# elisabeth96/nerf-rs

Hardware: AMD Instinct MI355X
Metric: rays/sec, lego 800x800 (64 coarse + 128 fine samples per ray) (higher is better)
Workload: dtype f32

## Files before the change

### bindings/rust/nerf-mi355x-sys/src/lib.rs

```rust
#![allow(non_camel_case_types)]
use std::os::raw::{c_char, c_int, c_void};

#[repr(C)]
pub struct nerf_ctx {
    _private: [u8; 0],
}

#[repr(C)]
#[derive(Clone, Copy, Debug, Default)]
pub struct nerf_camera {
    pub nx: i32,
    pub ny: i32,
    pub alpha_width: f32,
    pub alpha_height: f32,
    pub pos: [f32; 3],
    pub dir: [f32; 3],
    pub up: [f32; 3],
    pub near: f32,
    pub far: f32,
}

pub const NERF_MLP_F32: i32 = 0;
pub const NERF_MLP_BF16: i32 = 1;
pub const NERF_MLP_BF16X3: i32 = 2;
// ... 102 lines not shown
    pub fn nerf_pack_network_dir(dir: *const c_char, blob_path: *const c_char) -> c_int;
    pub fn nerf_load_network_blob(ctx: *mut nerf_ctx, which: c_int, blob_path: *const c_char) -> c_int;
    pub fn nerf_debug_pack_network_dir(dir: *const c_char, wstream: *mut f32, wstream_cap: usize, small: *mut f32,
                                       small_cap: usize, wstream_len: *mut usize, small_len: *mut usize) -> c_int;
    pub fn nerf_debug_fold_network_dir(dir: *const c_char, wstream: *mut f32, wstream_cap: usize, small: *mut f32,
                                       small_cap: usize, wstream_len: *mut usize, small_len: *mut usize) -> c_int;
    pub fn nerf_debug_network_stream_dir(dir: *const c_char, kind: c_int, out: *mut u16, cap: usize, n: *mut usize, available: *mut c_int) -> c_int;
    pub fn nerf_debug_zero_skip_network_dir(dir: *const c_char, eligible: *mut c_int) -> c_int;
    pub fn nerf_debug_split_bf16x3(values: *const f32, n: usize, parts: *mut u16) -> c_int;
    pub fn nerf_debug_split_f16x2(values: *const f32, n: usize, parts: *mut u16) -> c_int;
    pub fn nerf_debug_certify_policy(margin: f32, audited: u64, violations: u64, headroom: f32, max_error: f32, new_margin: *mut f32) -> c_int;
    pub fn nerf_debug_ray_grouping(n_rays: c_int, samples_per_ray: c_int, enabled: c_int, first_slot_of_wave_tile: *mut i32) -> c_int;
    pub fn nerf_debug_wave_tiling(rows: c_int, rays_per_row: c_int, samples_per_ray: c_int, full: c_int, ray_grouping: c_int, wave_tiling: c_int,
                                  slot: *mut i32) -> c_int;
    pub fn nerf_debug_tile_rotation(n_tiles: c_int, n_workgroups: c_int, rotation: c_int, workgroup_of_tile: *mut i32, round_of_tile: *mut i32) -> c_int;
    pub fn nerf_debug_shader_clock_mhz(ctx: *mut nerf_ctx, mhz: *mut f64) -> c_int;
    pub fn nerf_debug_workgroup_clocks(ctx: *mut nerf_ctx, out: *mut u64, n_workgroups: usize) -> c_int;
    pub fn nerf_forward_batch(ctx: *mut nerf_ctx, which: c_int, pts_soa: *const f32, dirs_aos: *const f32, n: usize,
                              rgb_aos: *mut f32, sigma: *mut f32) -> c_int;
    pub fn nerf_forward_batch_ex(ctx: *mut nerf_ctx, which: c_int, mlp_dtype: c_int, pts_soa: *const f32, dirs_aos: *const f32,
                                 n: usize, rgb_aos: *mut f32, sigma: *mut f32) -> c_int;
    pub fn nerf_forward_batch_device(ctx: *mut nerf_ctx, which: c_int, d_pts_soa: *const f32, d_dirs_aos: *const f32,
                                     n: usize, d_rgb_aos: *mut f32, d_sigma: *mut f32, stream: *mut c_void) -> c_int;
    pub fn nerf_density_batch(ctx: *mut nerf_ctx, which: c_int, pts_soa: *const f32, n: usize, sigma: *mut f32) -> c_int;
    pub fn nerf_density_batch_device(ctx: *mut nerf_ctx, which: c_int, d_pts_soa: *const f32, n: usize, d_sigma: *mut f32,
                                     stream: *mut c_void) -> c_int;
    pub fn nerf_density_grid(ctx: *mut nerf_ctx, which: c_int, lo: *const f32, step: *const f32, dims: *const i32, sigma_out: *mut f32,
                             threshold: f32, occ_bits: *mut u32, n_occupied: *mut u64, bounds: *mut i32) -> c_int;
    pub fn nerf_density_grid_device(ctx: *mut nerf_ctx, which: c_int, lo: *const f32, step: *const f32, dims: *const i32,
                                    d_sigma_out: *mut f32, threshold: f32, d_occ_bits: *mut u32, n_occupied: *mut u64, bounds: *mut i32,
// ... 176 lines not shown
```

### include/nerf_mi355x.h

```cpp
#ifndef NERF_MI355X_H
#define NERF_MI355X_H

#include <stddef.h>
#include <stdint.h>

#ifdef __cplusplus
extern "C" {
#endif

typedef struct nerf_ctx nerf_ctx;

typedef enum {
    NERF_OK = 0,
    NERF_ERR_INVALID = -1,
    NERF_ERR_IO = -2,
    NERF_ERR_MISSING = -3,
    NERF_ERR_SHAPE = -4,
    NERF_ERR_HIP = -5,
    NERF_ERR_STATE = -6,
    NERF_ERR_PARSE = -7
} nerf_status;

enum { NERF_NET_COARSE = 0, NERF_NET_FINE = 1 };
enum { NERF_MLP_F32 = 0, NERF_MLP_BF16 = 1, NERF_MLP_BF16X3 = 2, NERF_MLP_F16X2 = 3 };
// ... 58 lines not shown
int nerf_check_network_dir(const char *dir);
int nerf_check_network_blob(const char *blob_path);
int nerf_debug_pack_network_dir(const char *dir, float *wstream, size_t wstream_cap, float *small, size_t small_cap,
                                size_t *wstream_len, size_t *small_len);
int nerf_debug_fold_network_dir(const char *dir, float *wstream, size_t wstream_cap, float *small, size_t small_cap,
                                size_t *wstream_len, size_t *small_len);
enum { NERF_STREAM_BF16V2 = 0, NERF_STREAM_F16V2 = 1, NERF_STREAM_BF16X3 = 2, NERF_STREAM_F16X2 = 3 };
int nerf_debug_network_stream_dir(const char *dir, int kind, uint16_t *out, size_t cap, size_t *n, int *available);
int nerf_debug_zero_skip_network_dir(const char *dir, int *eligible);
int nerf_debug_split_bf16x3(const float *values, size_t n, uint16_t *parts );
int nerf_debug_certify_policy(float margin, uint64_t audited, uint64_t violations, float headroom, float max_error, float *new_margin);
int nerf_debug_split_f16x2(const float *values, size_t n, uint16_t *parts );
int nerf_debug_ray_grouping(int n_rays, int samples_per_ray, int enabled, int32_t *first_slot_of_wave_tile);
int nerf_debug_wave_tiling(int rows, int rays_per_row, int samples_per_ray, int full, int ray_grouping, int wave_tiling, int32_t *slot);
int nerf_debug_tile_rotation(int n_tiles, int n_workgroups, int rotation, int32_t *workgroup_of_tile, int32_t *round_of_tile);

int nerf_forward_batch(nerf_ctx *ctx, int which, const float *pts_soa , const float *dirs_aos ,
                       size_t n, float *rgb_aos , float *sigma );
int nerf_forward_batch_ex(nerf_ctx *ctx, int which, int mlp_dtype, const float *pts_soa, const float *dirs_aos, size_t n,
                          float *rgb_aos, float *sigma);
int nerf_forward_batch_device(nerf_ctx *ctx, int which, const float *d_pts_soa, const float *d_dirs_aos, size_t n,
                              float *d_rgb_aos, float *d_sigma, void *stream);

int nerf_density_batch(nerf_ctx *ctx, int which, const float *pts_soa , size_t n, float *sigma );
int nerf_density_batch_device(nerf_ctx *ctx, int which, const float *d_pts_soa, size_t n, float *d_sigma, void *stream);
int nerf_density_grid(nerf_ctx *ctx, int which, const float lo[3], const float step[3], const int32_t dims[3], float *sigma_out,
                      float threshold, uint32_t *occ_bits, uint64_t *n_occupied, int32_t bounds[6]);
int nerf_density_grid_device(nerf_ctx *ctx, int which, const float lo[3], const float step[3], const int32_t dims[3],
                             float *d_sigma_out, float threshold, uint32_t *d_occ_bits, uint64_t *n_occupied, int32_t bounds[6],
                             void *stream);
// ... 192 lines not shown
```

### nerf-rs_amd/_lib.py

```python
import ctypes as C
import os
import subprocess

_HERE = os.path.dirname(os.path.abspath(__file__))
_LIB = None

f32p = C.POINTER(C.c_float)
u8p = C.POINTER(C.c_uint8)
u32p = C.POINTER(C.c_uint32)
i32p = C.POINTER(C.c_int32)


class NerfError(RuntimeError):

    def __init__(self, code, msg):
        super().__init__(f"[{code}] {msg}")
        self.code = code
        self.msg = msg


class CCamera(C.Structure):
    _fields_ = [("nx", C.c_int32), ("ny", C.c_int32), ("alpha_width", C.c_float), ("alpha_height", C.c_float),
                ("pos", C.c_float * 3), ("dir", C.c_float * 3), ("up", C.c_float * 3),
                ("near", C.c_float), ("far", C.c_float)]
# ... 42 lines not shown
                                        C.POINTER(CCamera)]),
    "nerf_check_network_dir": (C.c_int, [C.c_char_p]),
    "nerf_check_network_blob": (C.c_int, [C.c_char_p]),
    "nerf_debug_pack_network_dir": (C.c_int, [C.c_char_p, f32p, C.c_size_t, f32p, C.c_size_t, C.POINTER(C.c_size_t),
                                              C.POINTER(C.c_size_t)]),
    "nerf_debug_fold_network_dir": (C.c_int, [C.c_char_p, f32p, C.c_size_t, f32p, C.c_size_t, C.POINTER(C.c_size_t),
                                              C.POINTER(C.c_size_t)]),
    "nerf_debug_network_stream_dir": (C.c_int, [C.c_char_p, C.c_int, C.POINTER(C.c_uint16), C.c_size_t, C.POINTER(C.c_size_t),
                                                C.POINTER(C.c_int)]),
    "nerf_debug_zero_skip_network_dir": (C.c_int, [C.c_char_p, C.POINTER(C.c_int)]),
    "nerf_debug_split_bf16x3": (C.c_int, [f32p, C.c_size_t, C.POINTER(C.c_uint16)]),
    "nerf_debug_split_f16x2": (C.c_int, [f32p, C.c_size_t, C.POINTER(C.c_uint16)]),
    "nerf_debug_certify_policy": (C.c_int, [C.c_float, C.c_uint64, C.c_uint64, C.c_float, C.c_float, f32p]),
    "nerf_debug_ray_grouping": (C.c_int, [C.c_int, C.c_int, C.c_int, C.POINTER(C.c_int32)]),
    "nerf_debug_tile_rotation": (C.c_int, [C.c_int, C.c_int, C.c_int, C.POINTER(C.c_int32), C.POINTER(C.c_int32)]),
    "nerf_debug_wave_tiling": (C.c_int, [C.c_int, C.c_int, C.c_int, C.c_int, C.c_int, C.c_int, C.POINTER(C.c_int32)]),
    "nerf_forward_batch": (C.c_int, [C.c_void_p, C.c_int, f32p, f32p, C.c_size_t, f32p, f32p]),
    "nerf_forward_batch_ex": (C.c_int, [C.c_void_p, C.c_int, C.c_int, f32p, f32p, C.c_size_t, f32p, f32p]),
    "nerf_forward_batch_device": (C.c_int, [C.c_void_p, C.c_int, C.c_void_p, C.c_void_p, C.c_size_t, C.c_void_p,
                                            C.c_void_p, C.c_void_p]),
    "nerf_density_batch": (C.c_int, [C.c_void_p, C.c_int, f32p, C.c_size_t, f32p]),
    "nerf_density_batch_device": (C.c_int, [C.c_void_p, C.c_int, C.c_void_p, C.c_size_t, C.c_void_p, C.c_void_p]),
    "nerf_density_grid": (C.c_int, [C.c_void_p, C.c_int, f32p, f32p, i32p, f32p, C.c_float, u32p, C.POINTER(C.c_uint64), i32p]),
    "nerf_density_grid_device": (C.c_int, [C.c_void_p, C.c_int, f32p, f32p, i32p, C.c_void_p, C.c_float, C.c_void_p,
                                           C.POINTER(C.c_uint64), i32p, C.c_void_p]),
    "nerf_isosurface_grid": (C.c_int, [C.c_void_p, f32p, f32p, f32p, i32p, C.c_float, f32p, f32p, C.c_size_t, u32p, C.c_size_t,
                                       C.POINTER(C.c_uint64), C.POINTER(C.c_uint64)]),
    "nerf_extract_mesh": (C.c_int, [C.c_void_p, C.c_int, f32p, f32p, i32p, C.c_float, f32p, f32p, f32p, C.c_size_t, u32p, C.c_size_t,
                                    C.POINTER(C.c_uint64), C.POINTER(C.c_uint64)]),
    "nerf_extract_mesh_device": (C.c_int, [C.c_void_p, C.c_int, f32p, f32p, i32p, C.c_float, C.c_void_p, C.c_void_p, C.c_void_p, C.c_size_t,
# ... 130 lines not shown
```

### nerf-rs_amd/csrc/mlp_kernel.h

```cpp
#pragma once
#include <hip/hip_runtime.h>

#include "mlp_layout.h"

enum { MLP_MODE_POINTS = 0, MLP_MODE_RAYS = 1, MLP_MODE_LIST = 2, MLP_MODE_GRID = 3 };

struct MlpArgs {
    const float *wstream;
    const float *small_params;
    int n_points;
    int mode;
    const float *pts_soa;
    const float *dirs_aos;
    const float *ray_dirs;
    const float *t;
    int samples_per_ray;
    float origin[3];
    float *sigma_out;
    float *rgb_out;
    int skip_empty;
    unsigned long long *skip_counter;
    unsigned long long *clock_out;
    unsigned int *nonfinite;
    int raw_pre;
// ... 4 lines not shown
    int grid_n[3];
    float occ_threshold;
    unsigned int *occ_bits;
    int zero_skip;
    unsigned long long *zskip_stats;
    int ray_grouping;
    int wave_tiling;
    int rays_per_row;
    nerfmlp::RayLaunchMap ray_map;
    const float *ray_origins;
    int depth_order;
    const unsigned int *order_table;
    int order_tiles, order_points;
    int tile_rotation;
    int empty_vote;
};

inline nerfmlp::DepthOrder nerf_mlp_depth_order(const MlpArgs &a, bool full) {
    return nerfmlp::depth_order_of(a.n_points, a.samples_per_ray, a.rays_per_row, full,
                                   a.mode == MLP_MODE_RAYS && a.depth_order != 0 && a.wave_tiling != 0 && a.skip_empty == 0);
}

hipError_t nerf_mlp_init();
hipError_t nerf_mlp_launch(const MlpArgs &a, bool full, int n_blocks, hipStream_t stream);
hipError_t nerf_zskip_clear(unsigned long long *stats, hipStream_t stream);
hipError_t nerf_zskip_print(const char *what, unsigned long long *stats, hipStream_t stream);
hipError_t nerf_mlp_bf16v2_init();
hipError_t nerf_mlp_bf16v2_launch(const MlpArgs &a, bool full, int n_blocks, hipStream_t stream);
hipError_t nerf_prefilter_f16v2_init();
hipError_t nerf_mlp_f16v2_launch(const MlpArgs &a, int n_blocks, hipStream_t stream);
struct SeqArgs;
// ... 57 lines not shown
```

### nerf-rs_amd/csrc/mlp_kernel.hip

```cpp
#include <hip/hip_runtime.h>
#include <stdint.h>
#include <stdio.h>

#include "mlp_f32_core.hip.h"
#include "mlp_kernel.h"

using namespace nerfmlp;
using namespace mlpdev;

using namespace mlpf32;

template <bool FULL, int MODE>
__global__ __launch_bounds__(256, 1) void nerf_mlp_kernel(const MlpArgs A) {
    extern __shared__ __attribute__((aligned(16))) char smem[];
    const LDS_AS char *lds = (const LDS_AS char *)smem;
    const LDS_AS float *small = (const LDS_AS float *)(lds + kRingSlots * kChunkBytes);

    const int tid = threadIdx.x;
    const int lane = tid & 63;
    const int wave = __builtin_amdgcn_readfirstlane(tid >> 6);
    const int p = lane & 31;
    const int h = lane >> 5;
    const int lane16 = lane * 16;

    {
        float *dst = (float *)(smem + kRingSlots * kChunkBytes);
        for (int i = tid; i < kSmallFloats; i += 256) dst[i] = A.small_params[i];
    }
// ... 25 lines not shown
    const int n_tiles = (n_points + kPointsPerBlock - 1) / kPointsPerBlock;
    constexpr int LOAD = (!FULL && MODE == MLP_MODE_POINTS) ? 4 : MODE;
    constexpr bool ORDER = FULL && MODE == MLP_MODE_RAYS;
    const int order_tiles = ORDER ? A.order_tiles : 0, order_points = ORDER ? A.order_points : 0;
    const int lane_part = (MODE == MLP_MODE_RAYS && A.ray_map.wt.ss) ? wave_tile_lane_part(A.ray_map.wt, p) : p;
    auto ordered = [&](int T) { return ORDER && T < order_tiles; };
    auto map_tile = [&](int T) { return ORDER ? max(T - order_tiles, 0) : T; };
    auto base_of = [&](int T) {
        return MODE == MLP_MODE_RAYS ? order_points + ray_launch_base(A.ray_map, map_tile(T), wave) : T * kPointsPerBlock + wave * kPointsPerWave;
    };
    auto lane_of = [&](int T) { return (MODE == MLP_MODE_RAYS && ray_launch_tiled(A.ray_map, map_tile(T))) ? lane_part : p; };
    auto entry_of = [&](int T) {
        return ordered(T) ? (int)min(A.order_table[(size_t)T * kPointsPerBlock + wave * kPointsPerWave + p], (unsigned)order_points - 1u) : 0;
    };
    const int G = gridDim.x;
    TileWalk walk = {0, 0};
    auto next_round_tile = [&]() { return tile_walk_next(walk, (int)blockIdx.x, G, A.tile_rotation != 0); };
    int tile_next = next_round_tile();
    int tile_next2 = next_round_tile();
    int base_next = base_of(blockIdx.x);
    int ord_cur = entry_of(blockIdx.x), ord_next = entry_of(tile_next);
    RawIn nxt = load_raw_at<LOAD>(A, ordered(blockIdx.x) ? ord_cur : base_next + lane_of(blockIdx.x));
    for (int tile = blockIdx.x; tile < n_tiles; tile = tile_next, tile_next = tile_next2, tile_next2 = next_round_tile()) {
        const int slot = ordered(tile) ? ord_cur : base_next + lane_of(tile);
        const bool valid = slot < n_points;
        base_next = base_of(tile_next);
        if (ORDER) { ord_cur = ord_next; ord_next = entry_of(tile_next2); }
        const RawIn in = nxt;
        nxt = load_raw_at<LOAD>(A, ordered(tile_next) ? ord_cur : base_next + lane_of(tile_next));
        float px, py, pz;
        point_of<MODE>(A, in, px, py, pz);
        const float dx = in.dx, dy = in.dy, dz = in.dz;
        const unsigned entry = __builtin_bit_cast(unsigned, in.b);
        const size_t i = MODE == MLP_MODE_LIST ? (size_t)(entry & 0x7fffffffu) : (size_t)slot;
        const bool audit = MODE == MLP_MODE_LIST && (entry >> 31) != 0;

        f32x16 E[2];
        encode_point(px, py, pz, h, E);

        f32x16 X[8], Y[8];

        load_bias<8>(X, small + kBiasOff + 0 * 256, h);
        tile_steps<8, false>(E[0], X, P);
        tile_steps<8, false>(E[1], X, P);
// ... 9 lines not shown
#pragma unroll
        for (int t = 0; t < 8; ++t) tile_steps<8, true>(X[t], Y, P);
        hidden_layer<true>(Y, X, small + kBiasOff + 6 * 256, P, h);
        hidden_layer<true>(X, Y, small + kBiasOff + 7 * 256, P, h);
        const float pre = alpha_pre(Y, small, h);
        sigma = fmaxf(pre, 0.f);
        if (MODE == MLP_MODE_GRID) {
            if (valid && h == 0 && A.sigma_out) A.sigma_out[i] = sigma;
            if (A.occ_bits) {
                const unsigned word = (unsigned)__ballot(valid && h == 0 && sigma > A.occ_threshold);
                const int slot0 = tile * kPointsPerBlock + wave * kPointsPerWave;
                if (lane == 0 && slot0 < n_points) A.occ_bits[slot0 >> 5] = word;
            }
        } else
        if (valid && h == 0) A.sigma_out[i] = audit ? pre : sigma;
        if (FULL && (A.skip_empty || A.empty_vote)) {
            LDS_AS int *vote = (LDS_AS int *)(lds + kRingSlots * kChunkBytes) + kMiscOff + 8;
            const bool any_wg = tile_has_density(vote, valid && sigma > 0.0f, wave, lane);
            if (!any_wg) {
                if (valid && h == 0) {
                    A.rgb_out[3 * (size_t)i + 0] = 0.f; A.rgb_out[3 * (size_t)i + 1] = 0.f; A.rgb_out[3 * (size_t)i + 2] = 0.f;
                }
                if (A.skip_counter && tid == 0) atomicAdd(A.skip_counter, 1ull);
                pipe_restart(P);
#if NERF_DIAG_RESTART_TWICE
                pipe_restart(P);
#endif
                continue;
            }
        }
// ... 22 lines not shown
    }
}

hipError_t nerf_zskip_clear(unsigned long long *stats, hipStream_t stream) {
    return stats ? hipMemsetAsync(stats, 0, 2 * sizeof(unsigned long long), stream) : hipSuccess;
}
hipError_t nerf_zskip_print(const char *what, unsigned long long *stats, hipStream_t stream) {
    if (!stats) return hipSuccess;
    unsigned long long h[2] = {0, 0};
    hipError_t e = hipMemcpyAsync(h, stats, sizeof h, hipMemcpyDeviceToHost, stream);
    if (e == hipSuccess) e = hipStreamSynchronize(stream);
    if (e == hipSuccess) fprintf(stderr, "nerf zskip: %s relu_ksteps_executed=%llu relu_ksteps_total=%llu\n", what, h[0], h[1]);
    return e;
}

template <bool FULL, int MODE>
static hipError_t launch_t(const MlpArgs &a, int n_blocks, hipStream_t stream) {
    hipError_t e = nerf_zskip_clear(a.zskip_stats, stream);
    if (e != hipSuccess) return e;
    hipLaunchKernelGGL((nerf_mlp_kernel<FULL, MODE>), dim3(n_blocks), dim3(256), kLdsBytes, stream, a);
    e = hipGetLastError();
    if (e != hipSuccess) return e;
    static const char *const modes[4] = {"points", "rays", "list", "grid"};
    char what[48];
    snprintf(what, sizeof what, "nerf_mlp_kernel<%s,%s>", FULL ? "full" : "sigma", modes[MODE]);
    return nerf_zskip_print(what, a.zskip_stats, stream);
}

hipError_t nerf_mlp_init() {
    const void *ks[7] = {(const void *)nerf_mlp_kernel<true, MLP_MODE_POINTS>, (const void *)nerf_mlp_kernel<true, MLP_MODE_RAYS>,
                         (const void *)nerf_mlp_kernel<false, MLP_MODE_RAYS>, (const void *)nerf_mlp_kernel<true, MLP_MODE_LIST>,
                         (const void *)nerf_mlp_kernel<false, MLP_MODE_LIST>, (const void *)nerf_mlp_kernel<false, MLP_MODE_POINTS>,
                         (const void *)nerf_mlp_kernel<false, MLP_MODE_GRID>};
    for (int i = 0; i < 7; ++i) {
        hipError_t e = hipFuncSetAttribute(ks[i], hipFuncAttributeMaxDynamicSharedMemorySize, kLdsBytes);
        if (e != hipSuccess) return e;
    }
    return hipSuccess;
}

static hipError_t launch_mlp_rays(const MlpArgs &a, bool full, int n_blocks, hipStream_t stream) {
    MlpArgs g = a;
    DepthOrder d = {0, 0, 0, 0};
    if (a.order_table) d = nerf_mlp_depth_order(a, full);
    g.order_tiles = d.tiles; g.order_points = d.points;
    if (!d.tiles) g.order_table = nullptr;
    g.ray_map = ray_launch_map_of(a.n_points - d.points, a.samples_per_ray, a.rays_per_row, full, a.ray_grouping != 0, a.wave_tiling != 0);
    return full ? launch_t<true, MLP_MODE_RAYS>(g, n_blocks, stream) : launch_t<false, MLP_MODE_RAYS>(g, n_blocks, stream);
}

hipError_t nerf_mlp_launch(const MlpArgs &a, bool full, int n_blocks, hipStream_t stream) {
    if (a.n_points <= 0) return hipSuccess;
    const int n_tiles = (a.n_points + kPointsPerBlock - 1) / kPointsPerBlock;
    if (n_blocks > n_tiles) n_blocks = n_tiles;
    if (n_blocks < 1) n_blocks = 1;
    if (a.mode == MLP_MODE_LIST) {
        if (!a.point_list || !a.point_list_count) return hipErrorInvalidValue;
        return full ? launch_t<true, MLP_MODE_LIST>(a, n_blocks, stream) : launch_t<false, MLP_MODE_LIST>(a, n_blocks, stream);
    }
    if (a.mode == MLP_MODE_GRID) {
        if (full || a.grid_n[0] <= 0 || a.grid_n[1] <= 0 || a.grid_n[2] <= 0 || (!a.sigma_out && !a.occ_bits)) return hipErrorInvalidValue;
        const unsigned long long plane = (unsigned long long)a.grid_n[0] * (unsigned long long)a.grid_n[1];
// ... 8 lines not shown
```

### nerf-rs_amd/csrc/mlp_layout.h

```cpp
#pragma once
#include <stdint.h>

namespace nerfmlp {

constexpr int kChunkBytes = 16384;
constexpr int kChunkFloats = kChunkBytes / 4;
#ifndef NERF_RING_SLOTS
#define NERF_RING_SLOTS 3
#endif
constexpr int kRingSlots = NERF_RING_SLOTS;
constexpr int kPointsPerWave = 32;
constexpr int kWavesPerBlock = 4;
constexpr int kPointsPerBlock = kPointsPerWave * kWavesPerBlock;

#if defined(__HIPCC__) || defined(__CUDACC__)
#define NERF_HOST_DEVICE __host__ __device__
#else
#define NERF_HOST_DEVICE
#endif
struct RayGrouping {
    int segments;
    int group_tiles;
};
NERF_HOST_DEVICE inline RayGrouping ray_grouping_of(int n_points, int samples_per_ray, bool allowed) {
// ... 107 lines not shown

NERF_HOST_DEVICE inline int rotated_tile(int k, int c, int G) {
    const int r = (int)((unsigned)(c + k % G) % (unsigned)G);
    return k * G + r;
}
struct TileWalk {
    int round_base, rot;
};
NERF_HOST_DEVICE inline int tile_walk_next(TileWalk &w, int c, int G, bool rotate) {
    w.round_base += G;
    if (rotate) w.rot = w.rot + 1 == G ? 0 : w.rot + 1;
    const int r = c + w.rot;
    return w.round_base + (r >= G ? r - G : r);
}

constexpr int kStepsL0 = 32;
constexpr int kStepsHid = 128;
constexpr int kStepsL5 = 160;
constexpr int kStepsView = 144;

constexpr int chunksOf(int steps, int nt) { return steps * nt * 256 / kChunkBytes; }

constexpr int kChunksSigma = chunksOf(kStepsL0, 8) + 4 * chunksOf(kStepsHid, 8) + chunksOf(kStepsL5, 8) +
                             2 * chunksOf(kStepsHid, 8);
constexpr int kChunksFull = kChunksSigma + chunksOf(kStepsHid, 8) + chunksOf(kStepsView, 4);

constexpr int kStepsViewFolded = kStepsHid + 16;
constexpr int kChunksColourFolded = chunksOf(kStepsViewFolded, 4);
constexpr int kChunksFullFolded = kChunksSigma + kChunksColourFolded;
constexpr int kFoldDirChunk = kChunksFull - 1;
// ... 52 lines not shown
```

### nerf-rs_amd/csrc/nerf_context.cpp

```cpp
#include <hip/hip_runtime.h>
#include <stdio.h>
#include <stdlib.h>

#include <algorithm>
#include <mutex>
#include <set>

#include "../../include/nerf_mi355x.h"
#include "host_util.h"
#include "mlp_kernel.h"
#include "sampling_kernels.h"

#include "nerf_internal.h"

namespace nerfint {

int fail(nerf_ctx *c, int code, const std::string &msg) {
    if (c) c->err = msg;
    return nerfhost::fail_noctx(code, msg);
}

hipEvent_t get_event(nerf_ctx *c) {
    if (!c->ev_pool.empty()) { hipEvent_t e = c->ev_pool.back(); c->ev_pool.pop_back(); return e; }
    hipEvent_t e = nullptr;
// ... 126 lines not shown
    if (const char *env = getenv("NERF_CERTIFY_AUDIT_MASK_NEAR")) { const long v = atol(env); if (v >= 0 && ((v + 1) & v) == 0) c->cert_audit_mask_near = (unsigned)v; }
    if (const char *env = getenv("NERF_CERTIFY_MARGINS")) {
        float m0 = 0.f, m1 = 0.f;
        if (sscanf(env, "%f,%f", &m0, &m1) == 2 && m0 > 0.f && m1 > 0.f) { c->cert_margin_floor[0] = m0; c->cert_margin_floor[1] = m1; c->cert_margin[0] = m0; c->cert_margin[1] = m1; }
    }
#endif
    env_size("NERF_GRADIENT_CHUNK", &c->gradient_chunk);
    if (const char *env = getenv("NERF_DEBUG_NORMALS")) c->debug_normals = atoi(env) > 0;
    if (const char *env = getenv("NERF_ZERO_STEP_SKIP")) c->zero_step_skip = atoi(env) != 0;
    if (const char *env = getenv("NERF_RAY_GROUPING")) c->ray_grouping = atoi(env) != 0;
    if (const char *env = getenv("NERF_WAVE_TILING")) c->wave_tiling = atoi(env) != 0;
    if (const char *env = getenv("NERF_DEPTH_ORDER")) c->depth_order = atoi(env) != 0;
    if (const char *env = getenv("NERF_TILE_ROTATION")) c->tile_rotation = atoi(env) != 0;
    if (const char *env = getenv("NERF_EMPTY_TILE_VOTE")) c->empty_tile_vote = atoi(env) != 0;
    if (const char *env = getenv("NERF_DEBUG_EMPTY_TILES")) c->debug_empty_tiles = atoi(env) > 0;
    if (const char *env = getenv("NERF_DEBUG_ZSKIP")) {
        if (atoi(env) > 0) {
            (void)c->buf[BUF_ZSKIP].ensure(c, 2 * sizeof(unsigned long long));
            c->empty_tile_vote = false;
        }
    }
    if (const char *env = getenv("NERF_DEBUG_CLOCK")) {
        if (atoi(env) > 0) (void)c->buf[BUF_CLOCK].ensure(c, (size_t)c->n_cus * 2 * sizeof(unsigned long long));
        c->clock_coarse = atoi(env) == 2;
    }
    (void)c->buf[BUF_SKIP].ensure(c, sizeof(unsigned long long));
    (void)c->buf[BUF_NONFINITE].ensure(c, sizeof(unsigned int));
    static std::mutex init_mu;
    static std::set<int> init_done;
    hipError_t e1 = hipSuccess, e2 = hipSuccess;
    {
        std::lock_guard<std::mutex> lk(init_mu);
        if (!init_done.count(device_id)) {
            e1 = init_mlp_kernels();
            e2 = e1 == hipSuccess ? sampling_init() : e1;
            if (e2 == hipSuccess) init_done.insert(device_id);
        }
    }
    hipError_t e3 = e2 == hipSuccess ? hipStreamCreate(&c->stream) : e2;
    if (e3 != hipSuccess) {
        const std::string m = std::string("context initialisation failed: ") + hipGetErrorString(e3);
        nerf_destroy(c);
// ... 79 lines not shown
```

### nerf-rs_amd/csrc/nerf_host_api.cpp

```cpp
#include <math.h>
#include <stdio.h>
#include <stdlib.h>
#include <string.h>

#include <map>
#include <new>
#include <string>
#include <vector>

#include "../../include/nerf_mi355x.h"
#include "host_util.h"
#include "mlp_layout.h"
#include "ray_clip_core.h"

using namespace nerfhost;

namespace nerfhost {

static thread_local std::string g_err;

int fail_noctx(int code, const std::string &msg) {
    g_err = msg;
    return code;
}
// ... 187 lines not shown
    if (n_tiles <= 0 || n_workgroups <= 0 || !workgroup_of_tile || !round_of_tile) return fail_noctx(NERF_ERR_INVALID, "n_tiles and n_workgroups must be > 0, the tables not NULL");
    if ((long long)n_tiles + 2ll * n_workgroups > INT32_MAX) return fail_noctx(NERF_ERR_INVALID, "too many tiles");
    for (int t = 0; t < n_tiles; ++t) workgroup_of_tile[t] = round_of_tile[t] = -1;
    for (int c = 0; c < n_workgroups; ++c) {
        TileWalk w = {0, 0};
        int k = 0;
        for (int tile = c; tile < n_tiles; tile = tile_walk_next(w, c, n_workgroups, rotation != 0), ++k) {
            if (rotation && tile != rotated_tile(k, c, n_workgroups)) return fail_noctx(NERF_ERR_INVALID, "internal error: the walk left rotated_tile");
            workgroup_of_tile[tile] = workgroup_of_tile[tile] == -1 ? c : -2;
            round_of_tile[tile] = k;
        }
    }
    return NERF_OK;
} NERF_HOST_CATCH

int nerf_debug_clip_rays(const uint32_t *occ_bits, const float lo[3], const float step[3], const int32_t dims[3], const float *origins,
                         size_t n_origins, const float *dirs, size_t n_rays, int normalize, float near_, float far_, const float *bounds,
                         float *bounds_out, uint8_t *hit_out, uint64_t *n_hit, uint64_t *n_refused_reads) try {
    const char *why = nerfclip::check_grid(occ_bits, lo, step, dims);
    if (!why) why = nerfclip::check_rays(origins, n_origins, dirs, n_rays, near_, far_, bounds, bounds_out, hit_out);
    if (why) return fail_noctx(NERF_ERR_INVALID, why);
    uint64_t hits = 0, refused = 0;
    for (size_t r = 0; r < n_rays; ++r) {
        float near_r, far_r;
        const nerfclip::Result res = nerfclip::clip_batch_ray(occ_bits, lo, step, dims, origins, n_origins == 1 ? 0 : 1, dirs, normalize ? 1 : 0, near_, far_,
                                                              bounds, r, &near_r, &far_r);
        bounds_out[2 * r] = res.t_first; bounds_out[2 * r + 1] = res.t_last;
        hit_out[r] = res.hit ? 1 : 0;
        hits += res.hit ? 1 : 0; refused += res.refused;
    }
// ... 67 lines not shown
```

### nerf-rs_amd/csrc/nerf_internal.h

```cpp
#pragma once
#include <hip/hip_runtime.h>
#include <stddef.h>
#include <stdint.h>

#include <algorithm>
#include <exception>
#include <new>
#include <string>
#include <vector>

#include "../../include/nerf_mi355x.h"
#include "stage_layout.h"

struct MlpArgs;
struct SeqArgs;
struct ColourArgs;
struct RayGenArgs;

namespace nerfint {

constexpr float kCertMarginCoarse = 1.0f, kCertMarginFine = 3.0f;
constexpr float kCertMarginCoarseF16 = 0.25f, kCertMarginFineF16 = 0.5f;

enum EvKind {
// ... 51 lines not shown
    BUF_STENCIL,
    BUF_CLIP,
    BUF_SEQ,
    BUF_H8,
    BUF_SLOT_POINT,
    BUF_FLAG_LIST,
    BUF_POINT_LIST,
    BUF_CERT,
    BUF_JSTAR,
    BUF_CERT_AUX,
    BUF_ORDER,
    BUF_SKIP,
    BUF_NONFINITE,
    BUF_CLOCK,
    BUF_ZSKIP,
    BUF_COUNT
};

struct CertCounters {
    uint32_t list1_len, list2_len;
    uint32_t audited, violations, headroom_code, max_err_bits;
    uint32_t fallback_rays;
    uint32_t aux_count;
    uint32_t pf_ray_head;
    uint32_t list1_back_len;
    unsigned long long pf_samples;
    uint32_t range_left;
    uint32_t unused[3];
};
static_assert(sizeof(CertCounters) == 64 && offsetof(CertCounters, audited) == 8 && offsetof(CertCounters, max_err_bits) == 20 &&
// ... 33 lines not shown
    bool cert_zero_tiles = true;
    float cert_zero_frac = 0.1f;
    bool cert_seq_prefilter = true;
    double cert_list_frac = 0.5;
    float hybrid_tau = 1e-5f;
    size_t max_export_bytes = (size_t)16 << 30;
    bool clock_valid = false;
    bool clock_coarse = false;
    bool zero_step_skip = true;
    bool ray_grouping = true;
    bool wave_tiling = true;
    bool depth_order = true;
    bool tile_rotation = true;
    bool empty_tile_vote = true;
    bool debug_empty_tiles = false;
    size_t max_rays_per_pass = (size_t)1 << 20;
    std::vector<hipEvent_t> ev_pool;
    std::vector<nerfint::EvPair> last_render;
    std::vector<nerfint::EvPair> dominant;
};

namespace nerfint {

int fail(nerf_ctx *c, int code, const std::string &msg);

#define HIP_TRY(c, expr)                                                                                    \
    do {                                                                                                    \
        hipError_t _e = (expr);                                                                             \
        if (_e != hipSuccess)                                                                               \
            return fail((c), NERF_ERR_HIP, std::string(#expr) + ": " + hipGetErrorString(_e));              \
// ... 106 lines not shown
```

### nerf-rs_amd/csrc/nerf_render.cpp

```cpp
#include <hip/hip_runtime.h>
#include <stdio.h>
#include <string.h>

#include <algorithm>
#include <cmath>
#include <mutex>
#include <vector>

#include "../../include/nerf_mi355x.h"
#include "host_util.h"
#include "mlp_kernel.h"
#include "mlp_layout.h"
#include "normal_kernels.h"
#include "ray_batch_kernels.h"
#include "ray_clip_core.h"
#include "ray_clip_kernels.h"
#include "sampling_kernels.h"

using namespace nerfhost;

#include "nerf_internal.h"

using namespace nerfint;

// ... 265 lines not shown
    fill_net(c, net, dt, a);
    a.n_points = p.n_rays * spr; a.samples_per_ray = spr; a.t = t;
    a.rays_per_row = j.batch ? 0 : p.g.rw;
    a.sigma_out = sigma_out; a.rgb_out = rgb_out;
    a.skip_empty = j.skip_empty; a.skip_counter = j.skip_empty ? c->dev<unsigned long long>(BUF_SKIP) : nullptr;
    if (which == (c->clock_coarse ? NERF_NET_COARSE : NERF_NET_FINE)) a.clock_out = j.clock_out;
    if (j.certify) return cert_pass(c, j, p, a, net, which, dt, kind);
    bool full = rgb_out != nullptr;
    const bool voted = c->empty_tile_vote && full && a.mode == MLP_MODE_RAYS && !j.skip_empty && dt != NERF_MLP_BF16;
    a.empty_vote = voted ? 1 : 0;
    const bool count_votes = voted && c->debug_empty_tiles && c->buf[BUF_SKIP].p;
    if (count_votes) {
        a.skip_counter = c->dev<unsigned long long>(BUF_SKIP);
        HIP_TRY(c, hipMemsetAsync(a.skip_counter, 0, sizeof(unsigned long long), st));
    }
    if (p.origins) {
        if (!full && dt != NERF_MLP_F32) { full = true; a.rgb_out = c->dev(BUF_RGBF); }
        BatchPointsArgs q{};
        q.n_rays = p.n_rays; q.spr = spr; q.origins = p.origins; q.dirs = c->dev(BUF_DIRS); q.t = t;
        q.pts_soa = j.d_pts; q.dirs_aos = j.d_daos;
        a.pts_soa = j.d_pts; a.dirs_aos = j.d_daos;
        int rc;
        if ((rc = timed(c, st, EV_OTHER, 0, [&]() -> int { HIP_TRY(c, launch_batch_points(q, st)); return NERF_OK; }))) return rc;
    }
    if (dt == NERF_MLP_F32 && !p.origins) {
        const nerfmlp::DepthOrder d = nerf_mlp_depth_order(a, full);
        if (d.tiles > 0) {
            int rc;
            if ((rc = c->buf[BUF_ORDER].ensure(c, (size_t)d.points * sizeof(unsigned int)))) return rc;
            DepthOrderArgs q{};
            q.t = t; q.rw = a.rays_per_row; q.spr = spr; q.blocks_x = d.blocks_x; q.blocks = d.blocks; q.table = c->dev<unsigned int>(BUF_ORDER);
            if ((rc = timed(c, st, EV_OTHER, 0, [&]() -> int { HIP_TRY(c, launch_depth_order(q, st)); return NERF_OK; }))) return rc;
            a.order_table = c->dev<unsigned int>(BUF_ORDER);
        }
    }
    const int rc = timed(c, st, kind, (uint64_t)a.n_points, [&]() -> int { HIP_TRY(c, launch_mlp(c, dt, a, full, st)); return NERF_OK; });
    if (rc || !count_votes) return rc;
    unsigned long long tiles = 0;
    HIP_TRY(c, hipMemcpyAsync(&tiles, a.skip_counter, sizeof tiles, hipMemcpyDeviceToHost, st));
    HIP_TRY(c, hipStreamSynchronize(st));
    static const char *const kernels[4] = {"nerf_mlp_kernel<full,rays>", "", "nerf_mlp_kernel_bf16x3<full,rays>", "nerf_mlp_kernel_f16x2<full,rays>"};
    fprintf(stderr, "nerf empty tiles: %s tiles_skipped=%llu tiles=%d\n", kernels[dt], tiles, (a.n_points + nerfmlp::kPointsPerBlock - 1) / nerfmlp::kPointsPerBlock);
    return NERF_OK;
}

int hybrid_redo(nerf_ctx *c, const RenderJob &j, const Pass &p, const ResampleArgs &ra, SeqCounters *hctr) {
    const hipStream_t st = j.st;
    const DevNet &NC = c->net[NERF_NET_COARSE];
    SeqArgs q = seq_args(c, j, p, j.nc, c->dev(BUF_TC), c->dev(BUF_SC));
    fill_net(c, NC, NERF_MLP_F32, q);
    q.ray_counter = &hctr->ray_head; q.stats = &hctr->evaluated;
// ... 801 lines not shown
```

### nerf-rs_amd/csrc/sampling_kernels.hip

```cpp
#include <hip/hip_runtime.h>
#include <stdint.h>

#include "philox.hip.h"
#include "sampling_kernels.h"

namespace {

__device__ __forceinline__ void wave_sync() {
    __builtin_amdgcn_fence(__ATOMIC_ACQ_REL, "wavefront");
    __builtin_amdgcn_wave_barrier();
}

}

__device__ __forceinline__ int ray_row(const RayGenArgs &a, int r) {
    const int j = a.ry0 + r / a.rw;
    return a.stripe > 0 ? a.stripe_y0 + ((j / a.stripe) * a.stripe_n + a.stripe_i) * a.stripe + j % a.stripe : j;
}

__global__ void k_ray_dirs(RayGenArgs a, float *__restrict__ dirs) {
    const int r = blockIdx.x * blockDim.x + threadIdx.x;
    if (r >= a.n_rays) return;
    const int i = ray_row(a, r), j = a.rx0 + r % a.rw;
    const float x = (((float)j + a.half) / (float)a.rnx) * 2.0f - 1.0f;
// ... 36 lines not shown
    bool cut = false, near = false;
#pragma unroll 8
    for (int i = 0; i < n; ++i) {
        const float al = alpha[i];
        const float wi = cut ? 0.0f : T * al;
        if (lane == 0) w[i] = wi;
        T = cut ? T : T * (1.0f - al);
        if (Tn && lane == 0) Tn[i] = T;
        near = near || fabsf(T - 1e-4f) < 1e-7f;
        cut = cut || T < 1e-4f;
    }
    return near;
}

__device__ __forceinline__ float sample_alpha(const float *t, const float *sigma, int i, int n, float far_) {
    float delta = (i + 1 < n) ? t[i + 1] - t[i] : far_ - t[i];
    if (delta < 0.0f) delta = 0.0f;
    return 1.0f - expf(-sigma[i] * delta);
}

__global__ __launch_bounds__(256) void k_resample(ResampleArgs a) {
    extern __shared__ __attribute__((aligned(16))) float lds_f[];
    const int lane = threadIdx.x & 63, wv = threadIdx.x >> 6;
    int ray = blockIdx.x * 4 + wv;
    if (ray >= a.n_rays) return;
    if (a.ray_list) {
        if ((unsigned)ray >= *a.ray_list_count) return;
        ray = (int)a.ray_list[ray];
    }
    const int nc = a.nc, nf = a.nf, M = nc + nf;
    float *t = lds_f + (size_t)wv * (7 * nc + a.sort_pow2);
    float *sg = t + nc, *alpha = sg + nc, *w = alpha + nc, *cdf = w + nc, *bins = cdf + nc, *Tn = bins + nc, *mg = Tn + nc;
    const bool flagging = a.flag_list || a.flag_out;
// ... 668 lines not shown
```

Measured before the change: 801,300.

## Cut coarse sigma MLP tiles once ray transmittance saturates

Adds a CUT variant of the sigma-only ray-mode MLP kernel. Each workgroup walks all tiles of one block of rays in depth order, accumulates transmittance across waves through LDS, and once every ray in the block is opaque it zero-fills the remaining sigma samples and jumps to the next unit taken from an atomic counter. This skips coarse-network evaluation of samples behind opaque surfaces, at the cost of an extra barrier, expf and LDS exchange per tile, plus serialised in-unit tile order that may reduce prefetch overlap and load balance. It is enabled by default when there are enough blocks per CU.

```diff
diff --git a/bindings/rust/nerf-mi355x-sys/src/lib.rs b/bindings/rust/nerf-mi355x-sys/src/lib.rs
--- a/bindings/rust/nerf-mi355x-sys/src/lib.rs
+++ b/bindings/rust/nerf-mi355x-sys/src/lib.rs
@@ -140,6 +140,8 @@
     pub fn nerf_debug_wave_tiling(rows: c_int, rays_per_row: c_int, samples_per_ray: c_int, full: c_int, ray_grouping: c_int, wave_tiling: c_int,
                                   slot: *mut i32) -> c_int;
     pub fn nerf_debug_tile_rotation(n_tiles: c_int, n_workgroups: c_int, rotation: c_int, workgroup_of_tile: *mut i32, round_of_tile: *mut i32) -> c_int;
+    pub fn nerf_debug_coarse_cut_walk(rows: c_int, rays_per_row: c_int, samples_per_ray: c_int, ray_grouping: c_int, cut_block: c_int, cut_after: c_int,
+                                      tiles: *mut i32, tiles_cap: usize, blocks: *mut i32, block_tiles: *mut i32) -> c_int;
     pub fn nerf_debug_shader_clock_mhz(ctx: *mut nerf_ctx, mhz: *mut f64) -> c_int;
     pub fn nerf_debug_workgroup_clocks(ctx: *mut nerf_ctx, out: *mut u64, n_workgroups: usize) -> c_int;
     pub fn nerf_forward_batch(ctx: *mut nerf_ctx, which: c_int, pts_soa: *const f32, dirs_aos: *const f32, n: usize,
diff --git a/include/nerf_mi355x.h b/include/nerf_mi355x.h
--- a/include/nerf_mi355x.h
+++ b/include/nerf_mi355x.h
@@ -96,6 +96,8 @@
 int nerf_debug_ray_grouping(int n_rays, int samples_per_ray, int enabled, int32_t *first_slot_of_wave_tile);
 int nerf_debug_wave_tiling(int rows, int rays_per_row, int samples_per_ray, int full, int ray_grouping, int wave_tiling, int32_t *slot);
 int nerf_debug_tile_rotation(int n_tiles, int n_workgroups, int rotation, int32_t *workgroup_of_tile, int32_t *round_of_tile);
+int nerf_debug_coarse_cut_walk(int rows, int rays_per_row, int samples_per_ray, int ray_grouping, int cut_block, int cut_after, int32_t *tiles,
+                               size_t tiles_cap, int32_t *blocks, int32_t *block_tiles);
 
 int nerf_forward_batch(nerf_ctx *ctx, int which, const float *pts_soa , const float *dirs_aos ,
                        size_t n, float *rgb_aos , float *sigma );
diff --git a/nerf-rs_amd/_lib.py b/nerf-rs_amd/_lib.py
--- a/nerf-rs_amd/_lib.py
+++ b/nerf-rs_amd/_lib.py
@@ -80,6 +80,8 @@
     "nerf_debug_certify_policy": (C.c_int, [C.c_float, C.c_uint64, C.c_uint64, C.c_float, C.c_float, f32p]),
     "nerf_debug_ray_grouping": (C.c_int, [C.c_int, C.c_int, C.c_int, C.POINTER(C.c_int32)]),
     "nerf_debug_tile_rotation": (C.c_int, [C.c_int, C.c_int, C.c_int, C.POINTER(C.c_int32), C.POINTER(C.c_int32)]),
+    "nerf_debug_coarse_cut_walk": (C.c_int, [C.c_int, C.c_int, C.c_int, C.c_int, C.c_int, C.c_int, C.POINTER(C.c_int32), C.c_size_t,
+                                            C.POINTER(C.c_int32), C.POINTER(C.c_int32)]),
     "nerf_debug_wave_tiling": (C.c_int, [C.c_int, C.c_int, C.c_int, C.c_int, C.c_int, C.c_int, C.POINTER(C.c_int32)]),
     "nerf_forward_batch": (C.c_int, [C.c_void_p, C.c_int, f32p, f32p, C.c_size_t, f32p, f32p]),
     "nerf_forward_batch_ex": (C.c_int, [C.c_void_p, C.c_int, C.c_int, f32p, f32p, C.c_size_t, f32p, f32p]),
diff --git a/nerf-rs_amd/csrc/mlp_kernel.h b/nerf-rs_amd/csrc/mlp_kernel.h
--- a/nerf-rs_amd/csrc/mlp_kernel.h
+++ b/nerf-rs_amd/csrc/mlp_kernel.h
@@ -42,7 +42,17 @@
     int order_tiles, order_points;
     int tile_rotation;
     int empty_vote;
+    int ray_cut;
+    float ray_cut_far;
+    unsigned int *cut_counters;
+    int cut_count;
 };
+
+inline nerfmlp::RayCutWalk nerf_mlp_ray_cut(const MlpArgs &a, bool full) {
+    if (full || a.mode != MLP_MODE_RAYS || !a.cut_counters) return nerfmlp::RayCutWalk{0, 0, 0, 0};
+    const nerfmlp::RayLaunchMap m = nerfmlp::ray_launch_map_of(a.n_points, a.samples_per_ray, a.rays_per_row, false, a.ray_grouping != 0, a.wave_tiling != 0);
+    return nerfmlp::ray_cut_walk_of(nerfmlp::ray_cut_map_of(m), a.n_points);
+}
 
 inline nerfmlp::DepthOrder nerf_mlp_depth_order(const MlpArgs &a, bool full) {
     return nerfmlp::depth_order_of(a.n_points, a.samples_per_ray, a.rays_per_row, full,
diff --git a/nerf-rs_amd/csrc/mlp_kernel.hip b/nerf-rs_amd/csrc/mlp_kernel.hip
--- a/nerf-rs_amd/csrc/mlp_kernel.hip
+++ b/nerf-rs_amd/csrc/mlp_kernel.hip
@@ -4,14 +4,16 @@
 
 #include "mlp_f32_core.hip.h"
 #include "mlp_kernel.h"
+#include "sample_alpha.hip.h"
 
 using namespace nerfmlp;
 using namespace mlpdev;
 
 using namespace mlpf32;
 
-template <bool FULL, int MODE>
+template <bool FULL, int MODE, bool CUT = false>
 __global__ __launch_bounds__(256, 1) void nerf_mlp_kernel(const MlpArgs A) {
+    static_assert(!CUT || (!FULL && MODE == MLP_MODE_RAYS), "the coarse cut belongs to the sigma-only ray-mode launch");
     extern __shared__ __attribute__((aligned(16))) char smem[];
     const LDS_AS char *lds = (const LDS_AS char *)smem;
     const LDS_AS float *small = (const LDS_AS float *)(lds + kRingSlots * kChunkBytes);
@@ -67,20 +69,42 @@
         return ordered(T) ? (int)min(A.order_table[(size_t)T * kPointsPerBlock + wave * kPointsPerWave + p], (unsigned)order_points - 1u) : 0;
     };
     const int G = gridDim.x;
+    RayCutWalk cw = {0, 0, 0, 0};
+    int unit = (int)blockIdx.x, unit_next = G + (int)blockIdx.x, unit_next2 = 0;
+    bool unit_first = true, cdone = false;
+    float cT = 1.0f, t_end_next = 0.f;
+    unsigned unit_asked = 0;
+    LDS_AS float *xch = (LDS_AS float *)(smem + kLdsBytes);
+    if constexpr (CUT) cw = ray_cut_walk_of(A.ray_map, n_points);
+    auto t_end_of = [&](int T_, int u_, int slot_) -> float {
+        if (T_ >= cw.rest_first) return 0.f;
+        const int s = (T_ - u_ * cw.block_tiles) * kWavesPerBlock + wave;
+        return s + 1 < A.samples_per_ray ? A.t[slot_ + 1] : A.ray_cut_far;
+    };
+    const int tile0 = CUT ? ray_cut_unit_tile(cw, unit, n_tiles) : (int)blockIdx.x;
     TileWalk walk = {0, 0};
     auto next_round_tile = [&]() { return tile_walk_next(walk, (int)blockIdx.x, G, A.tile_rotation != 0); };
     int tile_next = next_round_tile();
     int tile_next2 = next_round_tile();
-    int base_next = base_of(blockIdx.x);
-    int ord_cur = entry_of(blockIdx.x), ord_next = entry_of(tile_next);
-    RawIn nxt = load_raw_at<LOAD>(A, ordered(blockIdx.x) ? ord_cur : base_next + lane_of(blockIdx.x));
-    for (int tile = blockIdx.x; tile < n_tiles; tile = tile_next, tile_next = tile_next2, tile_next2 = next_round_tile()) {
+    int base_next = base_of(tile0);
+    int ord_cur = entry_of(tile0), ord_next = entry_of(tile_next);
+    RawIn nxt = load_raw_at<LOAD>(A, ordered(tile0) ? ord_cur : base_next + lane_of(tile0));
+    if constexpr (CUT) t_end_next = t_end_of(tile0, unit, base_next + lane_of(tile0));
+    for (int tile = tile0; tile < n_tiles; tile = tile_next, tile_next = tile_next2, tile_next2 = next_round_tile()) {
+        if constexpr (CUT) {
+            const int in_unit = ray_cut_next_in_unit(cw, unit, tile, false);
+            tile_next = in_unit >= 0 ? in_unit : ray_cut_unit_tile(cw, unit_next, n_tiles);
+            if (unit_first && tid == 0) unit_asked = atomicAdd(A.cut_counters, 1u);
+        }
         const int slot = ordered(tile) ? ord_cur : base_next + lane_of(tile);
         const bool valid = slot < n_points;
         base_next = base_of(tile_next);
         if (ORDER) { ord_cur = ord_next; ord_next = entry_of(tile_next2); }
         const RawIn in = nxt;
         nxt = load_raw_at<LOAD>(A, ordered(tile_next) ? ord_cur : base_next + lane_of(tile_next));
+        const float t_end = t_end_next;
+        if constexpr (CUT)
+            t_end_next = t_end_of(tile_next, ray_cut_next_in_unit(cw, unit, tile, false) >= 0 ? unit : unit_next, base_next + lane_of(tile_next));
         float px, py, pz;
         point_of<MODE>(A, in, px, py, pz);
         const float dx = in.dx, dy = in.dy, dz = in.dz;
@@ -120,6 +144,36 @@
             }
         } else
         if (valid && h == 0) A.sigma_out[i] = audit ? pre : sigma;
+        if constexpr (CUT) {
+            const float al = sample_alpha_of(in.a, t_end, sigma);
+            LDS_AS unsigned *xch_unit = (LDS_AS unsigned *)(xch + kPointsPerBlock);
+            if (h == 0) xch[wave * kPointsPerWave + p] = al;
+            if (unit_first && tid == 0) *xch_unit = unit_asked;
+            asm volatile("s_waitcnt lgkmcnt(0)\n\ts_barrier" ::: "memory");
+            if (unit_first)
+                unit_next2 = (int)min(2u * (unsigned)G + (unsigned)__builtin_amdgcn_readfirstlane((int)*xch_unit), (unsigned)ray_cut_units(cw));
+            bool all_cut = false;
+            if (tile < cw.rest_first) {
+#pragma unroll
+                for (int w = 0; w < kWavesPerBlock; ++w) transmittance_step(cT, cdone, xch[w * kPointsPerWave + p]);
+                all_cut = __all(cdone || !valid) != 0;
+            }
+            if (ray_cut_next_in_unit(cw, unit, tile, all_cut) < 0) {
+                const int end = (unit + 1) * cw.block_tiles;
+                if (all_cut && tile + 1 < end) {
+                    const int s0 = (tile + 1 - unit * cw.block_tiles) * kWavesPerBlock;
+                    float *row = A.sigma_out + (wave_tile_base_slot(A.ray_map.wt, unit * cw.block_tiles, 0) + wave_tile_lane_part(A.ray_map.wt, tid >> 3));
+                    for (int s = s0 + (tid & 7); s < A.samples_per_ray; s += 8) row[s] = 0.f;
+                    if (A.cut_count && tid == 0) atomicAdd((unsigned long long *)(A.cut_counters + 2), (unsigned long long)(end - tile - 1));
+                    tile_next = ray_cut_unit_tile(cw, unit_next, n_tiles);
+                    base_next = base_of(tile_next);
+                    nxt = load_raw_at<LOAD>(A, base_next + lane_of(tile_next));
+                    t_end_next = t_end_of(tile_next, unit_next, base_next + lane_of(tile_next));
+                }
+                unit = unit_next; unit_next = unit_next2; unit_first = true;
+                cT = 1.0f; cdone = false;
+            } else unit_first = false;
+        }
         if (FULL && (A.skip_empty || A.empty_vote)) {
             LDS_AS int *vote = (LDS_AS int *)(lds + kRingSlots * kChunkBytes) + kMiscOff + 8;
             const bool any_wg = tile_has_density(vote, valid && sigma > 0.0f, wave, lane);
@@ -172,11 +226,11 @@
     return e;
 }
 
-template <bool FULL, int MODE>
-static hipError_t launch_t(const MlpArgs &a, int n_blocks, hipStream_t stream) {
+template <bool FULL, int MODE, bool CUT = false>
+static hipError_t launch_t(const MlpArgs &a, int n_blocks, hipStream_t stream, int lds_bytes = kLdsBytes) {
     hipError_t e = nerf_zskip_clear(a.zskip_stats, stream);
     if (e != hipSuccess) return e;
-    hipLaunchKernelGGL((nerf_mlp_kernel<FULL, MODE>), dim3(n_blocks), dim3(256), kLdsBytes, stream, a);
+    hipLaunchKernelGGL((nerf_mlp_kernel<FULL, MODE, CUT>), dim3(n_blocks), dim3(256), lds_bytes, stream, a);
     e = hipGetLastError();
     if (e != hipSuccess) return e;
     static const char *const modes[4] = {"points", "rays", "list", "grid"};
@@ -186,12 +240,12 @@
 }
 
 hipError_t nerf_mlp_init() {
-    const void *ks[7] = {(const void *)nerf_mlp_kernel<true, MLP_MODE_POINTS>, (const void *)nerf_mlp_kernel<true, MLP_MODE_RAYS>,
+    const void *ks[8] = {(const void *)nerf_mlp_kernel<true, MLP_MODE_POINTS>, (const void *)nerf_mlp_kernel<true, MLP_MODE_RAYS>,
                          (const void *)nerf_mlp_kernel<false, MLP_MODE_RAYS>, (const void *)nerf_mlp_kernel<true, MLP_MODE_LIST>,
                          (const void *)nerf_mlp_kernel<false, MLP_MODE_LIST>, (const void *)nerf_mlp_kernel<false, MLP_MODE_POINTS>,
-                         (const void *)nerf_mlp_kernel<false, MLP_MODE_GRID>};
-    for (int i = 0; i < 7; ++i) {
-        hipError_t e = hipFuncSetAttribute(ks[i], hipFuncAttributeMaxDynamicSharedMemorySize, kLdsBytes);
+                         (const void *)nerf_mlp_kernel<false, MLP_MODE_GRID>, (const void *)nerf_mlp_kernel<false, MLP_MODE_RAYS, true>};
+    for (int i = 0; i < 8; ++i) {
+        hipError_t e = hipFuncSetAttribute(ks[i], hipFuncAttributeMaxDynamicSharedMemorySize, kLdsBytes + (i == 7 ? kCutLdsBytes : 0));
         if (e != hipSuccess) return e;
     }
     return hipSuccess;
@@ -204,6 +258,18 @@
     g.order_tiles = d.tiles; g.order_points = d.points;
     if (!d.tiles) g.order_table = nullptr;
     g.ray_map = ray_launch_map_of(a.n_points - d.points, a.samples_per_ray, a.rays_per_row, full, a.ray_grouping != 0, a.wave_tiling != 0);
+    g.ray_cut = 0;
+    if (a.ray_cut) {
+        const RayCutWalk w = nerf_mlp_ray_cut(a, full);
+        if (w.blocks > 0) {
+            g.ray_cut = 1;
+            g.ray_map = ray_cut_map_of(g.ray_map);
+            if (n_blocks > ray_cut_units(w)) n_blocks = ray_cut_units(w);
+            const hipError_t e = hipMemsetAsync(a.cut_counters, 0, sizeof(unsigned int), stream);
+            if (e != hipSuccess) return e;
+            return launch_t<false, MLP_MODE_RAYS, true>(g, n_blocks, stream, kLdsBytes + kCutLdsBytes);
+        }
+    }
     return full ? launch_t<true, MLP_MODE_RAYS>(g, n_blocks, stream) : launch_t<false, MLP_MODE_RAYS>(g, n_blocks, stream);
 }
 
diff --git a/nerf-rs_amd/csrc/mlp_layout.h b/nerf-rs_amd/csrc/mlp_layout.h
--- a/nerf-rs_amd/csrc/mlp_layout.h
+++ b/nerf-rs_amd/csrc/mlp_layout.h
@@ -145,6 +145,36 @@
     return w.round_base + (r >= G ? r - G : r);
 }
 
+struct RayCutWalk {
+    int blocks;
+    int block_tiles;
+    int rest_first;
+    int rest_tiles;
+};
+NERF_HOST_DEVICE inline RayLaunchMap ray_cut_map_of(RayLaunchMap m) {
+    m.wt.segments = 0; m.wt.group_tiles = 0;
+    return m;
+}
+NERF_HOST_DEVICE inline RayCutWalk ray_cut_walk_of(const RayLaunchMap &m, int n_points) {
+    RayCutWalk w = {0, 0, 0, 0};
+    if (m.wt.ss != 1 || m.wt.tw != kWaveTileSigmaW || m.wt.th != kWaveTileSigmaH || m.wt.segments != 0 || m.wt.spr % kWavesPerBlock != 0 || m.wt.tiled_tiles <= 0) return w;
+    w.block_tiles = m.wt.spr / kWavesPerBlock;
+    w.blocks = m.wt.tiled_tiles / w.block_tiles;
+    w.rest_first = m.wt.tiled_tiles;
+    w.rest_tiles = (n_points + kPointsPerBlock - 1) / kPointsPerBlock - m.wt.tiled_tiles;
+    return w;
+}
+NERF_HOST_DEVICE inline int ray_cut_units(const RayCutWalk &w) { return w.blocks + w.rest_tiles; }
+NERF_HOST_DEVICE inline int ray_cut_unit_tile(const RayCutWalk &w, int u, int n_tiles) {
+    if (u < w.blocks) return u * w.block_tiles;
+    return u - w.blocks < w.rest_tiles ? w.rest_first + (u - w.blocks) : n_tiles;
+}
+NERF_HOST_DEVICE inline int ray_cut_next_in_unit(const RayCutWalk &w, int u, int tile, bool all_cut) {
+    if (u >= w.blocks || all_cut) return -1;
+    return tile + 1 < (u + 1) * w.block_tiles ? tile + 1 : -1;
+}
+constexpr int kCutLdsBytes = (kPointsPerBlock + 4) * 4;
+
 constexpr int kStepsL0 = 32;
 constexpr int kStepsHid = 128;
 constexpr int kStepsL5 = 160;
diff --git a/nerf-rs_amd/csrc/nerf_context.cpp b/nerf-rs_amd/csrc/nerf_context.cpp
--- a/nerf-rs_amd/csrc/nerf_context.cpp
+++ b/nerf-rs_amd/csrc/nerf_context.cpp
@@ -164,10 +164,13 @@
     if (const char *env = getenv("NERF_TILE_ROTATION")) c->tile_rotation = atoi(env) != 0;
     if (const char *env = getenv("NERF_EMPTY_TILE_VOTE")) c->empty_tile_vote = atoi(env) != 0;
     if (const char *env = getenv("NERF_DEBUG_EMPTY_TILES")) c->debug_empty_tiles = atoi(env) > 0;
+    if (const char *env = getenv("NERF_COARSE_CUT")) c->coarse_cut = atoi(env) <= 0 ? 0 : atoi(env) >= 2 ? 2 : 1;
+    if (const char *env = getenv("NERF_DEBUG_COARSE_CUT")) c->debug_coarse_cut = atoi(env) > 0;
     if (const char *env = getenv("NERF_DEBUG_ZSKIP")) {
         if (atoi(env) > 0) {
             (void)c->buf[BUF_ZSKIP].ensure(c, 2 * sizeof(unsigned long long));
             c->empty_tile_vote = false;
+            c->coarse_cut = 0;
         }
     }
     if (const char *env = getenv("NERF_DEBUG_CLOCK")) {
@@ -176,6 +179,7 @@
     }
     (void)c->buf[BUF_SKIP].ensure(c, sizeof(unsigned long long));
     (void)c->buf[BUF_NONFINITE].ensure(c, sizeof(unsigned int));
+    if (c->coarse_cut) (void)c->buf[BUF_CUT].ensure(c, 2 * sizeof(unsigned long long));
     static std::mutex init_mu;
     static std::set<int> init_done;
     hipError_t e1 = hipSuccess, e2 = hipSuccess;
diff --git a/nerf-rs_amd/csrc/nerf_host_api.cpp b/nerf-rs_amd/csrc/nerf_host_api.cpp
--- a/nerf-rs_amd/csrc/nerf_host_api.cpp
+++ b/nerf-rs_amd/csrc/nerf_host_api.cpp
@@ -225,6 +225,31 @@
     return NERF_OK;
 } NERF_HOST_CATCH
 
+int nerf_debug_coarse_cut_walk(int rows, int rays_per_row, int samples_per_ray, int ray_grouping, int cut_block, int cut_after, int32_t *tiles,
+                               size_t tiles_cap, int32_t *blocks, int32_t *block_tiles) try {
+    using namespace nerfmlp;
+    if (rows <= 0 || rays_per_row <= 0 || samples_per_ray <= 0 || !tiles) return fail_noctx(NERF_ERR_INVALID, "rows, rays_per_row and samples_per_ray must be > 0, the table not NULL");
+    const long long n_points = (long long)rows * rays_per_row * samples_per_ray;
+    if (n_points > INT32_MAX - kPointsPerBlock) return fail_noctx(NERF_ERR_INVALID, "too many samples for one launch");
+    const int n = (int)n_points, n_tiles = (n + kPointsPerBlock - 1) / kPointsPerBlock;
+    if (tiles_cap < (size_t)n_tiles) return fail_noctx(NERF_ERR_INVALID, "the table holds fewer entries than the launch has tiles");
+    const RayCutWalk w = ray_cut_walk_of(ray_cut_map_of(ray_launch_map_of(n, samples_per_ray, rays_per_row, false, ray_grouping != 0, true)), n);
+    if (blocks) *blocks = w.blocks;
+    if (block_tiles) *block_tiles = w.block_tiles;
+    int visited = 0;
+    if (w.blocks == 0) {
+        for (int t = 0; t < n_tiles; ++t) tiles[visited++] = t;
+        return visited;
+    }
+    for (int u = 0; u < ray_cut_units(w); ++u)
+        for (int tile = ray_cut_unit_tile(w, u, n_tiles); tile >= 0 && tile < n_tiles;
+             tile = ray_cut_next_in_unit(w, u, tile, u == cut_block && tile - u * w.block_tiles >= cut_after)) {
+            if (visited >= n_tiles) return fail_noctx(NERF_ERR_INVALID, "internal error: the walk visits more tiles than the launch has");
+            tiles[visited++] = tile;
+        }
+    return visited;
+} NERF_HOST_CATCH
+
 int nerf_debug_clip_rays(const uint32_t *occ_bits, const float lo[3], const float step[3], const int32_t dims[3], const float *origins,
                          size_t n_origins, const float *dirs, size_t n_rays, int normalize, float near_, float far_, const float *bounds,
                          float *bounds_out, uint8_t *hit_out, uint64_t *n_hit, uint64_t *n_refused_reads) try {
diff --git a/nerf-rs_amd/csrc/nerf_internal.h b/nerf-rs_amd/csrc/nerf_internal.h
--- a/nerf-rs_amd/csrc/nerf_internal.h
+++ b/nerf-rs_amd/csrc/nerf_internal.h
@@ -89,6 +89,7 @@
     BUF_NONFINITE,
     BUF_CLOCK,
     BUF_ZSKIP,
+    BUF_CUT,
     BUF_COUNT
 };
 
@@ -152,6 +153,9 @@
     bool tile_rotation = true;
     bool empty_tile_vote = true;
     bool debug_empty_tiles = false;
+    static constexpr int kCutMinBlocksPerWorkgroup = 16;
+    int coarse_cut = 1;
+    bool debug_coarse_cut = false;
     size_t max_rays_per_pass = (size_t)1 << 20;
     std::vector<hipEvent_t> ev_pool;
     std::vector<nerfint::EvPair> last_render;
diff --git a/nerf-rs_amd/csrc/nerf_render.cpp b/nerf-rs_amd/csrc/nerf_render.cpp
--- a/nerf-rs_amd/csrc/nerf_render.cpp
+++ b/nerf-rs_amd/csrc/nerf_render.cpp
@@ -303,6 +303,18 @@
         a.skip_counter = c->dev<unsigned long long>(BUF_SKIP);
         HIP_TRY(c, hipMemsetAsync(a.skip_counter, 0, sizeof(unsigned long long), st));
     }
+    if (c->coarse_cut && c->buf[BUF_CUT].p && which == NERF_NET_COARSE && !full && dt == NERF_MLP_F32 && a.mode == MLP_MODE_RAYS && !j.batch &&
+        !j.coarse_only && j.nf > 0 && sigma_out == c->dev(BUF_SC)) {
+        a.cut_counters = c->dev<unsigned int>(BUF_CUT); a.ray_cut_far = j.far_;
+        const long long blocks = nerf_mlp_ray_cut(a, full).blocks;
+        a.ray_cut = blocks > 0 && (c->coarse_cut >= 2 || blocks >= (long long)nerf_ctx::kCutMinBlocksPerWorkgroup * c->n_cus) ? 1 : 0;
+        if (!a.ray_cut) a.cut_counters = nullptr;
+    }
+    const bool count_cut = a.ray_cut && c->debug_coarse_cut;
+    if (count_cut) {
+        a.cut_count = 1;
+        HIP_TRY(c, hipMemsetAsync(a.cut_counters + 2, 0, sizeof(unsigned long long), st));
+    }
     if (p.origins) {
         if (!full && dt != NERF_MLP_F32) { full = true; a.rgb_out = c->dev(BUF_RGBF); }
         BatchPointsArgs q{};
@@ -324,6 +336,13 @@
         }
     }
     const int rc = timed(c, st, kind, (uint64_t)a.n_points, [&]() -> int { HIP_TRY(c, launch_mlp(c, dt, a, full, st)); return NERF_OK; });
+    if (!rc && count_cut) {
+        unsigned long long skipped = 0;
+        HIP_TRY(c, hipMemcpyAsync(&skipped, a.cut_counters + 2, sizeof skipped, hipMemcpyDeviceToHost, st));
+        HIP_TRY(c, hipStreamSynchronize(st));
+        fprintf(stderr, "nerf coarse cut: nerf_mlp_kernel<sigma,rays> tiles_skipped=%llu tiles=%d blocks=%d\n", skipped,
+                (a.n_points + nerfmlp::kPointsPerBlock - 1) / nerfmlp::kPointsPerBlock, nerf_mlp_ray_cut(a, full).blocks);
+    }
     if (rc || !count_votes) return rc;
     unsigned long long tiles = 0;
     HIP_TRY(c, hipMemcpyAsync(&tiles, a.skip_counter, sizeof tiles, hipMemcpyDeviceToHost, st));
diff --git a/nerf-rs_amd/csrc/sample_alpha.hip.h b/nerf-rs_amd/csrc/sample_alpha.hip.h
--- /dev/null
+++ b/nerf-rs_amd/csrc/sample_alpha.hip.h
@@ -0,0 +1,13 @@
+#pragma once
+#include <hip/hip_runtime.h>
+
+__device__ __forceinline__ float sample_alpha_of(float t_cur, float t_end, float sigma) {
+    float delta = t_end - t_cur;
+    if (delta < 0.0f) delta = 0.0f;
+    return 1.0f - expf(-sigma * delta);
+}
+
+__device__ __forceinline__ void transmittance_step(float &T, bool &cut, float alpha) {
+    T = cut ? T : T * (1.0f - alpha);
+    cut = cut || T < 1e-4f;
+}
diff --git a/nerf-rs_amd/csrc/sampling_kernels.hip b/nerf-rs_amd/csrc/sampling_kernels.hip
--- a/nerf-rs_amd/csrc/sampling_kernels.hip
+++ b/nerf-rs_amd/csrc/sampling_kernels.hip
@@ -2,6 +2,7 @@
 #include <stdint.h>
 
 #include "philox.hip.h"
+#include "sample_alpha.hip.h"
 #include "sampling_kernels.h"
 
 namespace {
@@ -74,9 +75,7 @@
 }
 
 __device__ __forceinline__ float sample_alpha(const float *t, const float *sigma, int i, int n, float far_) {
-    float delta = (i + 1 < n) ? t[i + 1] - t[i] : far_ - t[i];
-    if (delta < 0.0f) delta = 0.0f;
-    return 1.0f - expf(-sigma[i] * delta);
+    return sample_alpha_of(t[i], (i + 1 < n) ? t[i + 1] : far_, sigma[i]);
 }
 
 __global__ __launch_bounds__(256) void k_resample(ResampleArgs a) {
```

New measurement: 865,100 (median of 6 runs). 8.0% higher.
